# nv-tlabs/GEN3C

Measured on NVIDIA H100. Metric: denoise-steps/sec, 7B DiT, 121-frame 720p latent, higher is better.
Workload: dtype bf16

## Files before the change

### gen3c_b200/csrc/attn_wgmma.cu

```cuda
#include <cmath>
#include <cstdlib>

#include "kernels.h"

namespace g3c {

constexpr int ATT_THREADS = 384;
constexpr int ATT_TILE = ATT_ROWS_PER_CTA;
constexpr int ATT_HALF_BYTES = 128 * 128;
constexpr int ATT_TILE_BYTES = 2 * ATT_HALF_BYTES;
constexpr int ATT_STAGES = 2;
constexpr int ATT_SMEM = ATT_TILE_BYTES + ATT_STAGES * 2 * ATT_TILE_BYTES + 256 + 1024;
static_assert(ATT_SMEM <= 227 * 1024, "attention: Q + K/V rings exceed the 227 KB of shared memory per block");
static_assert(1 + 4 * ATT_STAGES + 3 <= 256 / 8, "attention: barriers exceed their 256-byte area");

struct AttnParams {
  int Lq, Lk, heads;
  int ldo;
  int vt_chunk_len;
  __nv_bfloat16* O;
  float scale_log2;
  const uint32_t* chunk_flags;
  uint32_t flag_seq;
  int first_chunk;
  unsigned long long peer_timeout_ns;
  unsigned long long* wait_ns;
  unsigned long long* trace;
};

static unsigned long long* g_attn_trace = nullptr;

#define ATT_TR(role, slot)                                                                                  \
  do {                                                                                                      \
    if constexpr (kTrace) {                                                                                 \
      if (blockIdx.x == 0 && blockIdx.y == 0 && j < 64 && (threadIdx.x % 128) == 0)                         \
        p.trace[((role) * 64 + j) * 8 + (slot)] = clock64();                                                \
    }                                                                                                       \
  } while (0)

__device__ __forceinline__ float ex2_approx(float x) {
  float y;
  asm("ex2.approx.ftz.f32 %0, %1;\n" : "=f"(y) : "f"(x));
  return y;
}

__device__ __forceinline__ void softmax_tile(float (&s)[64], float (&m_run)[2], float (&l_run)[2], float (&alpha)[2],
                                             float sl2) {
  float mx[2] = {-INFINITY, -INFINITY};
#pragma unroll
  for (int i = 0; i < 16; ++i) {
    mx[0] = fmaxf(mx[0], fmaxf(s[4 * i], s[4 * i + 1]));
    mx[1] = fmaxf(mx[1], fmaxf(s[4 * i + 2], s[4 * i + 3]));
  }
  float nm[2];
#pragma unroll
  for (int h = 0; h < 2; ++h) {
    mx[h] = fmaxf(mx[h], __shfl_xor_sync(0xffffffffu, mx[h], 1));
    mx[h] = fmaxf(mx[h], __shfl_xor_sync(0xffffffffu, mx[h], 2));
    nm[h] = fmaxf(m_run[h], mx[h] * sl2);
    alpha[h] = ex2_approx(m_run[h] - nm[h]);
    m_run[h] = nm[h];
    l_run[h] *= alpha[h];
  }
#pragma unroll
  for (int i = 0; i < 16; ++i) {
    s[4 * i] = ex2_approx(fmaf(s[4 * i], sl2, -nm[0]));
    s[4 * i + 1] = ex2_approx(fmaf(s[4 * i + 1], sl2, -nm[0]));
    s[4 * i + 2] = ex2_approx(fmaf(s[4 * i + 2], sl2, -nm[1]));
    s[4 * i + 3] = ex2_approx(fmaf(s[4 * i + 3], sl2, -nm[1]));
    l_run[0] += s[4 * i] + s[4 * i + 1];
    l_run[1] += s[4 * i + 2] + s[4 * i + 3];
  }
}

__device__ __forceinline__ void issue_s(float (&s)[64], uint64_t dq, const uint8_t* k_tile) {
  const uint64_t dk = make_sdesc_sw128(smem_u32(k_tile));
#pragma unroll
  for (int kk = 0; kk < 8; ++kk) {
    const uint32_t off = (kk >> 2) * ATT_HALF_BYTES + (kk & 3) * 32;
    wgmma_ss_n128(s, sdesc_advance(dq, off), sdesc_advance(dk, off), kk > 0 ? 1u : 0u);
  }
}

template <bool kVTokenMajor>
__device__ __forceinline__ void issue_pv(float (&o)[64], const uint32_t (&pa)[32], const uint8_t* v_tile) {
  if constexpr (kVTokenMajor) {
    const uint64_t dv = make_sdesc_sw128_mn(smem_u32(v_tile), ATT_HALF_BYTES);
#pragma unroll
    for (int kk = 0; kk < 8; ++kk) {
      const uint32_t a[4] = {pa[4 * kk], pa[4 * kk + 1], pa[4 * kk + 2], pa[4 * kk + 3]};
      wgmma_rs_n128_tb(o, a, sdesc_advance(dv, kk * 16 * 128));
    }
  } else {
    const uint64_t dv = make_sdesc_sw128(smem_u32(v_tile));
#pragma unroll
    for (int kk = 0; kk < 8; ++kk) {
      const uint32_t a[4] = {pa[4 * kk], pa[4 * kk + 1], pa[4 * kk + 2], pa[4 * kk + 3]};
      wgmma_rs_n128(o, a, sdesc_advance(dv, (kk >> 2) * ATT_HALF_BYTES + (kk & 3) * 32));
    }
  }
}

__device__ __forceinline__ void mask_key_tail(float (&s)[64], int valid, uint32_t lane) {
#pragma unroll
  for (int i = 0; i < 16; ++i) {
    const int col = 8 * i + 2 * (int)(lane % 4);
    if (col >= valid) s[4 * i] = s[4 * i + 2] = -INFINITY;
    if (col + 1 >= valid) s[4 * i + 1] = s[4 * i + 3] = -INFINITY;
  }
}

__device__ __forceinline__ void pack_p(uint32_t (&pa)[32], const float (&s)[64]) {
#pragma unroll
  for (int i = 0; i < 16; ++i) {
    pa[2 * i] = pack_bf16x2(s[4 * i], s[4 * i + 1]);
    pa[2 * i + 1] = pack_bf16x2(s[4 * i + 2], s[4 * i + 3]);
  }
}

template <bool kTrace, bool kVTokenMajor = false>
__global__ void __launch_bounds__(ATT_THREADS, 1)
    k_attn_fwd(const __grid_constant__ CUtensorMap tmQ, const __grid_constant__ CUtensorMap tmK,
               const __grid_constant__ CUtensorMap tmV, const AttnParams p) {
  extern __shared__ uint8_t smem_raw[];
  uint8_t* smem = reinterpret_cast<uint8_t*>((reinterpret_cast<uintptr_t>(smem_raw) + 1023) &
                                             ~static_cast<uintptr_t>(1023));
  uint8_t* smem_q = smem;
  uint8_t* smem_k = smem + ATT_TILE_BYTES;
  uint8_t* smem_v = smem_k + ATT_STAGES * ATT_TILE_BYTES;
  uint64_t* bars = reinterpret_cast<uint64_t*>(smem_v + ATT_STAGES * ATT_TILE_BYTES);
  uint64_t* q_full = bars;
  uint64_t* k_full = bars + 1;
  uint64_t* v_full = k_full + ATT_STAGES;
  uint64_t* k_empty = v_full + ATT_STAGES;
  uint64_t* v_empty = k_empty + ATT_STAGES;
  uint64_t* turn = v_empty + ATT_STAGES;
  uint64_t* done = turn + 2;

  const uint32_t wg = threadIdx.x / 128;
  const uint32_t tid = threadIdx.x % 128;
  const int head = blockIdx.y;
  const int q0 = blockIdx.x * ATT_TILE;
  const int n_kv = kVTokenMajor ? (p.Lk + ATT_TILE - 1) / ATT_TILE : p.Lk / ATT_TILE;

  if (threadIdx.x == 0) {
    tma_prefetch_desc(&tmQ);
    tma_prefetch_desc(&tmK);
    tma_prefetch_desc(&tmV);
    mbar_init(q_full, 1);
    for (int i = 0; i < ATT_STAGES; ++i) {
      mbar_init(&k_full[i], 1);
      mbar_init(&v_full[i], 1);
      mbar_init(&k_empty[i], 2);
      mbar_init(&v_empty[i], 2);
    }
    for (int c = 0; c < 2; ++c) mbar_init(&turn[c], 4);
    for (int w = 0; w < 4; ++w) mbar_arrive(&turn[0]);
    mbar_init(done, 2);
    fence_barrier_init();
  }
  __syncthreads();

  if (wg == 0) {
    setmaxnreg_dec<24>();
    if (tid == 0) {
      mbar_expect_tx(q_full, ATT_TILE_BYTES);
      for (int h = 0; h < 2; ++h) tma_load_2d(smem_q + h * ATT_HALF_BYTES, &tmQ, q_full, head * 128 + h * 64, q0);
      const int tiles_per_chunk = p.vt_chunk_len / ATT_TILE;
      const int n_chunks = p.Lk / p.vt_chunk_len;
      uint32_t stage = 0, phase = 0;
      for (int j = 0; j < n_kv; ++j) {
        int chunk = 0, within = j;
        if constexpr (!kVTokenMajor) {
          chunk = p.first_chunk + j / tiles_per_chunk;
          if (chunk >= n_chunks) chunk -= n_chunks;
          within = j % tiles_per_chunk;
          if (p.chunk_flags && within == 0 && chunk != p.first_chunk) {
            uint32_t v, spins = 0;
            uint64_t t0 = 0;
            for (;;) {
              asm volatile("ld.acquire.sys.global.u32 %0, [%1];\n" : "=r"(v) : "l"(p.chunk_flags + chunk) : "memory");
              if ((int)(v - p.flag_seq) >= 0) break;
              if (t0 == 0) t0 = global_timer_ns();
              if ((++spins & 0x3FFu) == 0 && global_timer_ns() - t0 > p.peer_timeout_ns) asm volatile("trap;\n");
            }
            if (t0 != 0 && p.wait_ns) atomicAdd(p.wait_ns, (unsigned long long)(global_timer_ns() - t0));
            asm volatile("fence.proxy.async.global;\n" ::: "memory");
          }
        }
        const int kv0 = chunk * p.vt_chunk_len + within * ATT_TILE;
        mbar_wait_ns(&k_empty[stage], phase ^ 1, p.peer_timeout_ns);
        mbar_expect_tx(&k_full[stage], ATT_TILE_BYTES);
        for (int h = 0; h < 2; ++h)
          tma_load_2d(smem_k + stage * ATT_TILE_BYTES + h * ATT_HALF_BYTES, &tmK, &k_full[stage], head * 128 + h * 64,
                      kv0);
        mbar_wait_ns(&v_empty[stage], phase ^ 1, p.peer_timeout_ns);
        mbar_expect_tx(&v_full[stage], ATT_TILE_BYTES);
        for (int h = 0; h < 2; ++h) {
          if constexpr (kVTokenMajor)
            tma_load_2d(smem_v + stage * ATT_TILE_BYTES + h * ATT_HALF_BYTES, &tmV, &v_full[stage],
                        head * 128 + h * 64, kv0);
          else
            tma_load_3d(smem_v + stage * ATT_TILE_BYTES + h * ATT_HALF_BYTES, &tmV, &v_full[stage],
                        within * ATT_TILE + h * 64, head * 128, chunk);
        }
        if (++stage == ATT_STAGES) {
          stage = 0;
          phase ^= 1;
        }
      }
      mbar_wait_ns(done, 0, p.peer_timeout_ns);
    }
  } else {
    setmaxnreg_inc<240>();
    const uint32_t c = wg - 1;
    const uint32_t warp = tid / 32, lane = tid % 32;
    const unsigned long long tmo = p.peer_timeout_ns;
    float o[64];
#pragma unroll
    for (int i = 0; i < 64; ++i) o[i] = 0.f;
    float s[64];
    uint32_t pa[32];
    float m_run[2] = {-INFINITY, -INFINITY};
    float l_run[2] = {0.f, 0.f};
    float alpha[2];
    const float sl2 = p.scale_log2;
    const uint64_t dq = make_sdesc_sw128(smem_u32(smem_q + c * 64 * 128));
    uint32_t tph = 0;
    uint32_t ks = 0, kp = 0;
    uint32_t vs = 0, vp = 0;
    int j = 0;
    mbar_wait_ns_or_exit(q_full, 0, tmo);
    mbar_wait_ns_or_exit(&k_full[ks], kp, tmo);
    mbar_wait_ns_or_exit(&turn[c], tph, tmo);
    tph ^= 1;
    ATT_TR(1 + c, 0);
    wgmma_fence();
    issue_s(s, dq, smem_k + ks * ATT_TILE_BYTES);
    wgmma_commit();
    if (lane == 0) mbar_arrive(&turn[c ^ 1]);
    ATT_TR(1 + c, 1);
    wgmma_wait<0>();
    fence_regs(s);
    if (tid == 0) mbar_arrive(&k_empty[ks]);
    ATT_TR(1 + c, 2);
    if constexpr (kVTokenMajor) {
      if (n_kv == 1) mask_key_tail(s, p.Lk, lane);
    }
    softmax_tile(s, m_run, l_run, alpha, sl2);
    pack_p(pa, s);
    ATT_TR(1 + c, 3);
    if (++ks == ATT_STAGES) {
      ks = 0;
      kp ^= 1;
    }
    for (j = 1; j < (kVTokenMajor ? n_kv - 1 : n_kv); ++j) {
      mbar_wait_ns_or_exit(&k_full[ks], kp, tmo);
      mbar_wait_ns_or_exit(&v_full[vs], vp, tmo);
      mbar_wait_ns_or_exit(&turn[c], tph, tmo);
      tph ^= 1;
      ATT_TR(1 + c, 0);
      wgmma_fence();
      issue_s(s, dq, smem_k + ks * ATT_TILE_BYTES);
      wgmma_commit();
      issue_pv<kVTokenMajor>(o, pa, smem_v + vs * ATT_TILE_BYTES);
      wgmma_commit();
      if (lane == 0) mbar_arrive(&turn[c ^ 1]);
      ATT_TR(1 + c, 1);
      wgmma_wait<1>();
      fence_regs(s);
      if (tid == 0) mbar_arrive(&k_empty[ks]);
      ATT_TR(1 + c, 2);
      softmax_tile(s, m_run, l_run, alpha, sl2);
      ATT_TR(1 + c, 3);
      wgmma_wait<0>();
      fence_regs(o);
      fence_regs(pa);
      if (tid == 0) mbar_arrive(&v_empty[vs]);
      ATT_TR(1 + c, 4);
#pragma unroll
      for (int i = 0; i < 16; ++i) {
        o[4 * i] *= alpha[0];
        o[4 * i + 1] *= alpha[0];
        o[4 * i + 2] *= alpha[1];
        o[4 * i + 3] *= alpha[1];
      }
      pack_p(pa, s);
      if (++ks == ATT_STAGES) {
        ks = 0;
        kp ^= 1;
      }
      if (++vs == ATT_STAGES) {
        vs = 0;
        vp ^= 1;
      }
    }
    if constexpr (kVTokenMajor) {
      if (n_kv > 1) {
        mbar_wait_ns_or_exit(&k_full[ks], kp, tmo);
        mbar_wait_ns_or_exit(&v_full[vs], vp, tmo);
        mbar_wait_ns_or_exit(&turn[c], tph, tmo);
        tph ^= 1;
        ATT_TR(1 + c, 0);
        wgmma_fence();
        issue_s(s, dq, smem_k + ks * ATT_TILE_BYTES);
        wgmma_commit();
        issue_pv<kVTokenMajor>(o, pa, smem_v + vs * ATT_TILE_BYTES);
        wgmma_commit();
        if (lane == 0) mbar_arrive(&turn[c ^ 1]);
        ATT_TR(1 + c, 1);
        wgmma_wait<1>();
        fence_regs(s);
        if (tid == 0) mbar_arrive(&k_empty[ks]);
        ATT_TR(1 + c, 2);
        mask_key_tail(s, p.Lk - j * ATT_TILE, lane);
        softmax_tile(s, m_run, l_run, alpha, sl2);
        ATT_TR(1 + c, 3);
        wgmma_wait<0>();
        fence_regs(o);
        fence_regs(pa);
        if (tid == 0) mbar_arrive(&v_empty[vs]);
        ATT_TR(1 + c, 4);
#pragma unroll
        for (int i = 0; i < 16; ++i) {
          o[4 * i] *= alpha[0];
          o[4 * i + 1] *= alpha[0];
          o[4 * i + 2] *= alpha[1];
          o[4 * i + 3] *= alpha[1];
        }
        pack_p(pa, s);
        if (++vs == ATT_STAGES) {
          vs = 0;
          vp ^= 1;
        }
      }
      j = n_kv;
    }
    mbar_wait_ns_or_exit(&v_full[vs], vp, tmo);
    mbar_wait_ns_or_exit(&turn[c], tph, tmo);
    ATT_TR(1 + c, 0);
    wgmma_fence();
    issue_pv<kVTokenMajor>(o, pa, smem_v + vs * ATT_TILE_BYTES);
    wgmma_commit();
    if (lane == 0) mbar_arrive(&turn[c ^ 1]);
    ATT_TR(1 + c, 1);
    wgmma_wait<0>();
    fence_regs(o);
    fence_regs(pa);
    if (tid == 0) mbar_arrive(&v_empty[vs]);
    ATT_TR(1 + c, 4);
    float inv[2];
#pragma unroll
    for (int h = 0; h < 2; ++h) {
      float l = l_run[h];
      l += __shfl_xor_sync(0xffffffffu, l, 1);
      l += __shfl_xor_sync(0xffffffffu, l, 2);
      inv[h] = 1.0f / l;
    }
    const int row_a = q0 + (int)(c * 64 + warp * 16 + lane / 4);
#pragma unroll
    for (int h = 0; h < 2; ++h) {
      const int row = row_a + 8 * h;
      if (row >= p.Lq) continue;
      __nv_bfloat16* dst = p.O + (size_t)row * p.ldo + head * 128 + 2 * (lane % 4);
#pragma unroll
      for (int i = 0; i < 16; ++i)
        *reinterpret_cast<uint32_t*>(dst + 8 * i) = pack_bf16x2(o[4 * i + 2 * h] * inv[h], o[4 * i + 2 * h + 1] * inv[h]);
    }
    if (tid == 0) mbar_arrive(done);
  }
}

static int make_tmap_tokens(CUtensorMap* m, const void* base, int rows, int heads, int ld) {
  uint64_t dims[2] = {(uint64_t)heads * 128, (uint64_t)rows}, str[1] = {(uint64_t)ld * 2};
  uint32_t box[2] = {64, 128};
  return make_tmap_bf16_sw128(m, base, 2, dims, str, box);
}

static float scale_log2(float scale) {
  const float s = scale * 1.4426950408889634f;
  return fabsf(s - 1.0f) < 1e-6f ? 1.0f : s;
}

int attn_fwd(const void* q, const void* k, const void* vt, void* o, int Lq, int Lk, int heads,
             int ldq, int ldk, int ldo, int vt_chunk_len, float scale, cudaStream_t st, const ChunkGate* gate) {
  G3C_REQUIRE(q && k && vt && o, "attn: null operand");
  G3C_REQUIRE(Lq > 0 && Lk > 0 && heads > 0, "attn: bad sizes");
  G3C_REQUIRE(Lk % ATT_TILE == 0, "attn: Lk=%d must be a multiple of 128", Lk);
  if (vt_chunk_len <= 0) vt_chunk_len = Lk;
  G3C_REQUIRE(Lk % vt_chunk_len == 0 && vt_chunk_len % ATT_TILE == 0,
              "attn: vt_chunk_len=%d must divide Lk=%d and be a multiple of 128", vt_chunk_len, Lk);
  G3C_REQUIRE(ldq % 8 == 0 && ldk % 8 == 0 && ldo % 8 == 0 && ldq >= heads * 128 &&
                  ldk >= heads * 128 && ldo >= heads * 128,
              "attn: leading dimensions must be >= heads*128 and multiples of 8");
  G3C_REQUIRE((reinterpret_cast<uintptr_t>(o) & 15) == 0, "attn: O must be 16-byte aligned");
  CUtensorMap tmQ, tmK, tmV;
  int rc = make_tmap_tokens(&tmQ, q, Lq, heads, ldq);
  if (rc) return rc;
  rc = make_tmap_tokens(&tmK, k, Lk, heads, ldk);
  if (rc) return rc;
  {
    const int chunks = Lk / vt_chunk_len;
    uint64_t dims[3] = {(uint64_t)vt_chunk_len, (uint64_t)heads * 128, (uint64_t)chunks};
    uint64_t str[2] = {(uint64_t)vt_chunk_len * 2, (uint64_t)vt_chunk_len * 2 * heads * 128};
    uint32_t box[3] = {64, 128, 1};
    rc = make_tmap_bf16_sw128(&tmV, vt, 3, dims, str, box);
    if (rc) return rc;
  }
  static bool configured = false;
  if (!configured) {
    G3C_CUDA(cudaFuncSetAttribute(k_attn_fwd<false>, cudaFuncAttributeMaxDynamicSharedMemorySize, ATT_SMEM));
    G3C_CUDA(cudaFuncSetAttribute(k_attn_fwd<true>, cudaFuncAttributeMaxDynamicSharedMemorySize, ATT_SMEM));
    configured = true;
  }
  AttnParams p;
  p.Lq = Lq;
  p.Lk = Lk;
  p.heads = heads;
  p.ldo = ldo;
  p.vt_chunk_len = vt_chunk_len;
  p.O = reinterpret_cast<__nv_bfloat16*>(o);
  p.scale_log2 = scale_log2(scale);
  p.chunk_flags = gate ? gate->flags : nullptr;
  p.peer_timeout_ns = gate ? peer_timeout_ns() : G3C_MBAR_TIMEOUT_NS;
  p.wait_ns = gate ? gate->wait_ns : nullptr;
  p.flag_seq = gate ? gate->seq : 0;
  p.first_chunk = gate ? gate->first : 0;
  p.trace = g_attn_trace;
  G3C_REQUIRE(p.first_chunk >= 0 && p.first_chunk < Lk / vt_chunk_len, "attn: first chunk %d out of range", p.first_chunk);
  dim3 grid((Lq + ATT_TILE - 1) / ATT_TILE, heads);
  if (g_attn_trace) k_attn_fwd<true><<<grid, ATT_THREADS, ATT_SMEM, st>>>(tmQ, tmK, tmV, p);
  else k_attn_fwd<false><<<grid, ATT_THREADS, ATT_SMEM, st>>>(tmQ, tmK, tmV, p);
  G3C_CUDA(cudaGetLastError());
  return G3C_OK;
}

int attn_fwd_sbhd(const void* q, const void* k, const void* v, void* o, int Lq, int Lk, int batch, int heads, int ldq,
                  int ldk, int ldv, int ldo, float scale, cudaStream_t st) {
  G3C_REQUIRE(q && k && v && o, "attn_sbhd: null operand");
  G3C_REQUIRE(Lq > 0 && Lk > 0, "attn_sbhd: Lq=%d and Lk=%d must be >= 1", Lq, Lk);
  G3C_REQUIRE(batch > 0 && heads > 0 && (long long)batch * heads <= 65535,
              "attn_sbhd: batch=%d x heads=%d must be in [1, 65535]", batch, heads);
  const int bh = batch * heads;
  G3C_REQUIRE(ldq % 8 == 0 && ldk % 8 == 0 && ldv % 8 == 0 && ldo % 8 == 0 && ldq >= bh * 128 && ldk >= bh * 128 &&
                  ldv >= bh * 128 && ldo >= bh * 128,
              "attn_sbhd: leading dimensions (%d, %d, %d, %d) must be >= batch*heads*128 = %d and multiples of 8", ldq,
              ldk, ldv, ldo, bh * 128);
  G3C_REQUIRE(((reinterpret_cast<uintptr_t>(q) | reinterpret_cast<uintptr_t>(k) | reinterpret_cast<uintptr_t>(v) |
                reinterpret_cast<uintptr_t>(o)) & 15) == 0,
              "attn_sbhd: q, k, v and o must be 16-byte aligned");
  CUtensorMap tmQ, tmK, tmV;
  int rc = make_tmap_tokens(&tmQ, q, Lq, bh, ldq);
  if (rc) return rc;
  rc = make_tmap_tokens(&tmK, k, Lk, bh, ldk);
  if (rc) return rc;
  rc = make_tmap_tokens(&tmV, v, Lk, bh, ldv);
  if (rc) return rc;
  static bool configured = false;
  if (!configured) {
    G3C_CUDA(cudaFuncSetAttribute(k_attn_fwd<false, true>, cudaFuncAttributeMaxDynamicSharedMemorySize, ATT_SMEM));
    configured = true;
  }
  AttnParams p = {};
  p.Lq = Lq;
  p.Lk = Lk;
  p.heads = bh;
  p.ldo = ldo;
  p.vt_chunk_len = Lk;
  p.O = reinterpret_cast<__nv_bfloat16*>(o);
  p.scale_log2 = scale_log2(scale);
  p.peer_timeout_ns = G3C_MBAR_TIMEOUT_NS;
  dim3 grid((Lq + ATT_TILE - 1) / ATT_TILE, bh);
  k_attn_fwd<false, true><<<grid, ATT_THREADS, ATT_SMEM, st>>>(tmQ, tmK, tmV, p);
  G3C_CUDA(cudaGetLastError());
  return G3C_OK;
}

}

extern "C" int g3c_attn_set_trace(unsigned long long* device_buffer) {
  g3c::g_attn_trace = device_buffer;
  return G3C_OK;
}

extern "C" int g3c_attn_fwd(const void* q, const void* k, const void* vt, void* o, int Lq, int Lk,
                            int heads, int ldq, int ldk, int ldo, int vt_chunk_len, float scale,
                            void* stream) {
  return g3c::attn_fwd(q, k, vt, o, Lq, Lk, heads, ldq, ldk, ldo, vt_chunk_len, scale,
                       (cudaStream_t)stream, nullptr);
}

extern "C" int g3c_attn_fwd_sbhd(const void* q, const void* k, const void* v, void* o, int Lq, int Lk, int batch,
                                 int heads, int ldq, int ldk, int ldv, int ldo, float scale, void* stream) {
  return g3c::attn_fwd_sbhd(q, k, v, o, Lq, Lk, batch, heads, ldq, ldk, ldv, ldo, scale, (cudaStream_t)stream);
}
```

Baseline: 0.1297.

## Skip attention output rescale with lazy max threshold and unroll the KV ring loop

Softmax now keeps a reference max and only rescales the output accumulator and running sum when a warp's new max exceeds the reference by more than 8 in log2 space, skipping the per-tile multiply of 64 accumulators in most iterations. The consumer loop is unrolled for a two-stage ring with stage indices and parities derived statically, and shared-memory descriptors are precomputed as 32-bit low words to cut per-iteration descriptor arithmetic. The tail step is folded into the same lambda. This risks larger intermediate exponent values, with bf16 P values up to 2^8, and parity bookkeeping errors.

```diff
diff --git a/gen3c_b200/csrc/attn_wgmma.cu b/gen3c_b200/csrc/attn_wgmma.cu
--- a/gen3c_b200/csrc/attn_wgmma.cu
+++ b/gen3c_b200/csrc/attn_wgmma.cu
@@ -13,6 +13,8 @@
 constexpr int ATT_SMEM = ATT_TILE_BYTES + ATT_STAGES * 2 * ATT_TILE_BYTES + 256 + 1024;
 static_assert(ATT_SMEM <= 227 * 1024, "attention: Q + K/V rings exceed the 227 KB of shared memory per block");
 static_assert(1 + 4 * ATT_STAGES + 3 <= 256 / 8, "attention: barriers exceed their 256-byte area");
+static_assert(ATT_STAGES == 2, "attention: the consumer loop is unrolled for a ring depth of 2");
+constexpr float ATT_RESCALE_LOG2 = 8.0f;
 
 struct AttnParams {
   int Lq, Lk, heads;
@@ -44,7 +46,7 @@
   return y;
 }
 
-__device__ __forceinline__ void softmax_tile(float (&s)[64], float (&m_run)[2], float (&l_run)[2], float (&alpha)[2],
+__device__ __forceinline__ bool softmax_tile(float (&s)[64], float (&m_ref)[2], float (&l_run)[2], float (&alpha)[2],
                                              float sl2) {
   float mx[2] = {-INFINITY, -INFINITY};
 #pragma unroll
@@ -52,52 +54,57 @@
     mx[0] = fmaxf(mx[0], fmaxf(s[4 * i], s[4 * i + 1]));
     mx[1] = fmaxf(mx[1], fmaxf(s[4 * i + 2], s[4 * i + 3]));
   }
-  float nm[2];
 #pragma unroll
   for (int h = 0; h < 2; ++h) {
     mx[h] = fmaxf(mx[h], __shfl_xor_sync(0xffffffffu, mx[h], 1));
     mx[h] = fmaxf(mx[h], __shfl_xor_sync(0xffffffffu, mx[h], 2));
-    nm[h] = fmaxf(m_run[h], mx[h] * sl2);
-    alpha[h] = ex2_approx(m_run[h] - nm[h]);
-    m_run[h] = nm[h];
-    l_run[h] *= alpha[h];
-  }
+    mx[h] *= sl2;
+  }
+  const bool keep = __all_sync(0xffffffffu, mx[0] - m_ref[0] <= ATT_RESCALE_LOG2 && mx[1] - m_ref[1] <= ATT_RESCALE_LOG2);
+  if (!keep) {
+#pragma unroll
+    for (int h = 0; h < 2; ++h) {
+      const float nm = fmaxf(m_ref[h], mx[h]);
+      alpha[h] = ex2_approx(m_ref[h] - nm);
+      m_ref[h] = nm;
+      l_run[h] *= alpha[h];
+    }
+  }
+  const float nm0 = -m_ref[0], nm1 = -m_ref[1];
 #pragma unroll
   for (int i = 0; i < 16; ++i) {
-    s[4 * i] = ex2_approx(fmaf(s[4 * i], sl2, -nm[0]));
-    s[4 * i + 1] = ex2_approx(fmaf(s[4 * i + 1], sl2, -nm[0]));
-    s[4 * i + 2] = ex2_approx(fmaf(s[4 * i + 2], sl2, -nm[1]));
-    s[4 * i + 3] = ex2_approx(fmaf(s[4 * i + 3], sl2, -nm[1]));
+    s[4 * i] = ex2_approx(fmaf(s[4 * i], sl2, nm0));
+    s[4 * i + 1] = ex2_approx(fmaf(s[4 * i + 1], sl2, nm0));
+    s[4 * i + 2] = ex2_approx(fmaf(s[4 * i + 2], sl2, nm1));
+    s[4 * i + 3] = ex2_approx(fmaf(s[4 * i + 3], sl2, nm1));
     l_run[0] += s[4 * i] + s[4 * i + 1];
     l_run[1] += s[4 * i + 2] + s[4 * i + 3];
   }
-}
-
-__device__ __forceinline__ void issue_s(float (&s)[64], uint64_t dq, const uint8_t* k_tile) {
-  const uint64_t dk = make_sdesc_sw128(smem_u32(k_tile));
+  return !keep;
+}
+
+constexpr uint32_t ATT_SDESC_HI = (1024u >> 4) | (1u << 30);
+__device__ __forceinline__ uint64_t sdesc_at(uint32_t lo, uint32_t bytes) {
+  return (static_cast<uint64_t>(ATT_SDESC_HI) << 32) | (lo + (bytes >> 4));
+}
+
+__device__ __forceinline__ void issue_s(float (&s)[64], uint32_t dq, uint32_t dk) {
 #pragma unroll
   for (int kk = 0; kk < 8; ++kk) {
     const uint32_t off = (kk >> 2) * ATT_HALF_BYTES + (kk & 3) * 32;
-    wgmma_ss_n128(s, sdesc_advance(dq, off), sdesc_advance(dk, off), kk > 0 ? 1u : 0u);
+    wgmma_ss_n128(s, sdesc_at(dq, off), sdesc_at(dk, off), kk > 0 ? 1u : 0u);
   }
 }
 
 template <bool kVTokenMajor>
-__device__ __forceinline__ void issue_pv(float (&o)[64], const uint32_t (&pa)[32], const uint8_t* v_tile) {
-  if constexpr (kVTokenMajor) {
-    const uint64_t dv = make_sdesc_sw128_mn(smem_u32(v_tile), ATT_HALF_BYTES);
-#pragma unroll
-    for (int kk = 0; kk < 8; ++kk) {
-      const uint32_t a[4] = {pa[4 * kk], pa[4 * kk + 1], pa[4 * kk + 2], pa[4 * kk + 3]};
-      wgmma_rs_n128_tb(o, a, sdesc_advance(dv, kk * 16 * 128));
-    }
-  } else {
-    const uint64_t dv = make_sdesc_sw128(smem_u32(v_tile));
-#pragma unroll
-    for (int kk = 0; kk < 8; ++kk) {
-      const uint32_t a[4] = {pa[4 * kk], pa[4 * kk + 1], pa[4 * kk + 2], pa[4 * kk + 3]};
-      wgmma_rs_n128(o, a, sdesc_advance(dv, (kk >> 2) * ATT_HALF_BYTES + (kk & 3) * 32));
-    }
+__device__ __forceinline__ void issue_pv(float (&o)[64], const uint32_t (&pa)[32], uint32_t dv) {
+#pragma unroll
+  for (int kk = 0; kk < 8; ++kk) {
+    const uint32_t a[4] = {pa[4 * kk], pa[4 * kk + 1], pa[4 * kk + 2], pa[4 * kk + 3]};
+    if constexpr (kVTokenMajor)
+      wgmma_rs_n128_tb(o, a, sdesc_at(dv, kk * 16 * 128));
+    else
+      wgmma_rs_n128(o, a, sdesc_at(dv, (kk >> 2) * ATT_HALF_BYTES + (kk & 3) * 32));
   }
 }
 
@@ -213,7 +220,7 @@
     }
   } else {
     setmaxnreg_inc<240>();
-    const uint32_t c = wg - 1;
+    const uint32_t c = __shfl_sync(0xffffffffu, wg - 1, 0);
     const uint32_t warp = tid / 32, lane = tid % 32;
     const unsigned long long tmo = p.peer_timeout_ns;
     float o[64];
@@ -221,106 +228,63 @@
     for (int i = 0; i < 64; ++i) o[i] = 0.f;
     float s[64];
     uint32_t pa[32];
-    float m_run[2] = {-INFINITY, -INFINITY};
+    float m_ref[2] = {-INFINITY, -INFINITY};
     float l_run[2] = {0.f, 0.f};
     float alpha[2];
     const float sl2 = p.scale_log2;
-    const uint64_t dq = make_sdesc_sw128(smem_u32(smem_q + c * 64 * 128));
-    uint32_t tph = 0;
-    uint32_t ks = 0, kp = 0;
-    uint32_t vs = 0, vp = 0;
+    const uint32_t dq = (uint32_t)make_sdesc_sw128(smem_u32(smem_q + c * 64 * 128));
+    uint32_t dk[ATT_STAGES], dv[ATT_STAGES];
+#pragma unroll
+    for (int st = 0; st < ATT_STAGES; ++st) {
+      dk[st] = (uint32_t)make_sdesc_sw128(smem_u32(smem_k + st * ATT_TILE_BYTES));
+      dv[st] = (uint32_t)(kVTokenMajor ? make_sdesc_sw128_mn(smem_u32(smem_v + st * ATT_TILE_BYTES), ATT_HALF_BYTES)
+                                       : make_sdesc_sw128(smem_u32(smem_v + st * ATT_TILE_BYTES)));
+    }
     int j = 0;
     mbar_wait_ns_or_exit(q_full, 0, tmo);
-    mbar_wait_ns_or_exit(&k_full[ks], kp, tmo);
-    mbar_wait_ns_or_exit(&turn[c], tph, tmo);
-    tph ^= 1;
+    mbar_wait_ns_or_exit(&k_full[0], 0, tmo);
+    mbar_wait_ns_or_exit(&turn[c], 0, tmo);
     ATT_TR(1 + c, 0);
     wgmma_fence();
-    issue_s(s, dq, smem_k + ks * ATT_TILE_BYTES);
+    issue_s(s, dq, dk[0]);
     wgmma_commit();
     if (lane == 0) mbar_arrive(&turn[c ^ 1]);
     ATT_TR(1 + c, 1);
     wgmma_wait<0>();
     fence_regs(s);
-    if (tid == 0) mbar_arrive(&k_empty[ks]);
+    if (tid == 0) mbar_arrive(&k_empty[0]);
     ATT_TR(1 + c, 2);
     if constexpr (kVTokenMajor) {
       if (n_kv == 1) mask_key_tail(s, p.Lk, lane);
     }
-    softmax_tile(s, m_run, l_run, alpha, sl2);
+    softmax_tile(s, m_ref, l_run, alpha, sl2);
     pack_p(pa, s);
     ATT_TR(1 + c, 3);
-    if (++ks == ATT_STAGES) {
-      ks = 0;
-      kp ^= 1;
-    }
-    for (j = 1; j < (kVTokenMajor ? n_kv - 1 : n_kv); ++j) {
-      mbar_wait_ns_or_exit(&k_full[ks], kp, tmo);
-      mbar_wait_ns_or_exit(&v_full[vs], vp, tmo);
-      mbar_wait_ns_or_exit(&turn[c], tph, tmo);
-      tph ^= 1;
+    auto step = [&](int kst, int vst, uint32_t kpar, uint32_t vpar, int valid) {
+      mbar_wait_ns_or_exit(&k_full[kst], kpar, tmo);
+      mbar_wait_ns_or_exit(&v_full[vst], vpar, tmo);
+      mbar_wait_ns_or_exit(&turn[c], (uint32_t)j & 1u, tmo);
       ATT_TR(1 + c, 0);
       wgmma_fence();
-      issue_s(s, dq, smem_k + ks * ATT_TILE_BYTES);
+      issue_s(s, dq, kst ? dk[1] : dk[0]);
       wgmma_commit();
-      issue_pv<kVTokenMajor>(o, pa, smem_v + vs * ATT_TILE_BYTES);
+      issue_pv<kVTokenMajor>(o, pa, vst ? dv[1] : dv[0]);
       wgmma_commit();
       if (lane == 0) mbar_arrive(&turn[c ^ 1]);
       ATT_TR(1 + c, 1);
       wgmma_wait<1>();
       fence_regs(s);
-      if (tid == 0) mbar_arrive(&k_empty[ks]);
+      if (tid == 0) mbar_arrive(&k_empty[kst]);
       ATT_TR(1 + c, 2);
-      softmax_tile(s, m_run, l_run, alpha, sl2);
+      if (valid < ATT_TILE) mask_key_tail(s, valid, lane);
+      const bool rescale = softmax_tile(s, m_ref, l_run, alpha, sl2);
       ATT_TR(1 + c, 3);
       wgmma_wait<0>();
       fence_regs(o);
       fence_regs(pa);
-      if (tid == 0) mbar_arrive(&v_empty[vs]);
+      if (tid == 0) mbar_arrive(&v_empty[vst]);
       ATT_TR(1 + c, 4);
-#pragma unroll
-      for (int i = 0; i < 16; ++i) {
-        o[4 * i] *= alpha[0];
-        o[4 * i + 1] *= alpha[0];
-        o[4 * i + 2] *= alpha[1];
-        o[4 * i + 3] *= alpha[1];
-      }
-      pack_p(pa, s);
-      if (++ks == ATT_STAGES) {
-        ks = 0;
-        kp ^= 1;
-      }
-      if (++vs == ATT_STAGES) {
-        vs = 0;
-        vp ^= 1;
-      }
-    }
-    if constexpr (kVTokenMajor) {
-      if (n_kv > 1) {
-        mbar_wait_ns_or_exit(&k_full[ks], kp, tmo);
-        mbar_wait_ns_or_exit(&v_full[vs], vp, tmo);
-        mbar_wait_ns_or_exit(&turn[c], tph, tmo);
-        tph ^= 1;
-        ATT_TR(1 + c, 0);
-        wgmma_fence();
-        issue_s(s, dq, smem_k + ks * ATT_TILE_BYTES);
-        wgmma_commit();
-        issue_pv<kVTokenMajor>(o, pa, smem_v + vs * ATT_TILE_BYTES);
-        wgmma_commit();
-        if (lane == 0) mbar_arrive(&turn[c ^ 1]);
-        ATT_TR(1 + c, 1);
-        wgmma_wait<1>();
-        fence_regs(s);
-        if (tid == 0) mbar_arrive(&k_empty[ks]);
-        ATT_TR(1 + c, 2);
-        mask_key_tail(s, p.Lk - j * ATT_TILE, lane);
-        softmax_tile(s, m_run, l_run, alpha, sl2);
-        ATT_TR(1 + c, 3);
-        wgmma_wait<0>();
-        fence_regs(o);
-        fence_regs(pa);
-        if (tid == 0) mbar_arrive(&v_empty[vs]);
-        ATT_TR(1 + c, 4);
+      if (rescale) {
 #pragma unroll
         for (int i = 0; i < 16; ++i) {
           o[4 * i] *= alpha[0];
@@ -328,26 +292,37 @@
           o[4 * i + 2] *= alpha[1];
           o[4 * i + 3] *= alpha[1];
         }
-        pack_p(pa, s);
-        if (++vs == ATT_STAGES) {
-          vs = 0;
-          vp ^= 1;
-        }
+      }
+      pack_p(pa, s);
+    };
+    const int j_end = kVTokenMajor ? n_kv - 1 : n_kv;
+    uint32_t ph = 0;
+    for (j = 1; j < j_end; ++j) {
+      step(1, 0, ph, ph, ATT_TILE);
+      if (++j == j_end) break;
+      step(0, 1, ph ^ 1u, ph, ATT_TILE);
+      ph ^= 1u;
+    }
+    if constexpr (kVTokenMajor) {
+      if (n_kv > 1) {
+        j = n_kv - 1;
+        step(j & 1, (j - 1) & 1, ((uint32_t)j >> 1) & 1u, ((uint32_t)(j - 1) >> 1) & 1u, p.Lk - j * ATT_TILE);
       }
       j = n_kv;
     }
-    mbar_wait_ns_or_exit(&v_full[vs], vp, tmo);
-    mbar_wait_ns_or_exit(&turn[c], tph, tmo);
+    const int vst = (n_kv - 1) & 1;
+    mbar_wait_ns_or_exit(&v_full[vst], ((uint32_t)(n_kv - 1) >> 1) & 1u, tmo);
+    mbar_wait_ns_or_exit(&turn[c], (uint32_t)n_kv & 1u, tmo);
     ATT_TR(1 + c, 0);
     wgmma_fence();
-    issue_pv<kVTokenMajor>(o, pa, smem_v + vs * ATT_TILE_BYTES);
+    issue_pv<kVTokenMajor>(o, pa, vst ? dv[1] : dv[0]);
     wgmma_commit();
     if (lane == 0) mbar_arrive(&turn[c ^ 1]);
     ATT_TR(1 + c, 1);
     wgmma_wait<0>();
     fence_regs(o);
     fence_regs(pa);
-    if (tid == 0) mbar_arrive(&v_empty[vs]);
+    if (tid == 0) mbar_arrive(&v_empty[vst]);
     ATT_TR(1 + c, 4);
     float inv[2];
 #pragma unroll
```

New measurement: 0.1348 (median of 6 runs). +3.9%, better.
